# AKASH2907/pi-consistency-activity-detection

Hardware: AMD Instinct MI355X
Metric: train clips/sec (bs=8, 16×224×224, I3D+caps+bv cons) at 1/2/4/8 GPU (higher is better)
Workload: dtype f32 (fp32 operands and fp32 accumulation everywhere; 33 of the 79 conv / input-gradient launches and the 3x3x3 / 1x1x1 weight gradients multiply on the bf16 matrix cores: every fp32 operand as the exact sum of 3 bf16 terms, 6 products on v_mfma_f32_32x32x16_bf16, hi / lo fp32 accumulators -- error v

## Files before the change

pi-consistency-activity-detection_amd/csrc/caps.hip:

```cpp
#include "common.h"
#include <stdlib.h>

namespace {

constexpr int NB = 32;
constexpr int MAXC = 24;
constexpr int CJ = MAXC / 4;
constexpr float EPS = 1e-8f;
constexpr float LAMBDA = 1e-6f;
constexpr float HALF_LN_2PI = 0.91893853320467274178f;

#define WSYNC()                                               \
    do {                                                      \
        __builtin_amdgcn_fence(__ATOMIC_RELEASE, "workgroup"); \
        __builtin_amdgcn_wave_barrier();                      \
        __builtin_amdgcn_fence(__ATOMIC_ACQUIRE, "workgroup"); \
    } while (0)

template <int CTRL> __device__ __forceinline__ float dpp_mov(float v) {
    return __builtin_bit_cast(float, __builtin_amdgcn_update_dpp(0, __builtin_bit_cast(int, v), CTRL, 0xf, 0xf, true));
}
constexpr int DPP_XOR1 = 0xB1, DPP_XOR2 = 0x4E;
constexpr int DPP_HALF_MIRROR = 0x141, DPP_MIRROR = 0x140;
constexpr int DPP_ROR4 = 0x124, DPP_ROR8 = 0x128;
// ... 496 lines not shown
                    if (t < 2) is2[t][j] = 0.f;
                    if (c < C) {
                        dm[t][j] = bs->dmu[t][c][h]; dsv[t][j] = bs->ds2[t][c][h]; muv[t][j] = st->mu[t][c][h];
                        irs[t][j] = 1.0f / (st->rs[t][c] + EPS);
                        if (t < 2) is2[t][j] = 1.0f / st->s2[t][c][h];
                    }
                }
            float* dxp = dx + pos * (NB * 17);
            for (int i = i0; i < i1; ++i) {
                const f32x4 prow = *(const f32x4*)&st->P[i][p * 4];
                const float ai = st->a[i];
                f32x4 dP = {0.f, 0.f, 0.f, 0.f};
#pragma unroll
                for (int j = 0; j < CJ; ++j) {
                    const int c = cg + 4 * j;
                    if (c >= C) continue;
                    const f32x4 w = *(const f32x4*)(WT + ((i * C + c) * 4 + q) * 4);
                    const float v = prow[0] * w[0] + prow[1] * w[1] + prow[2] * w[2] + prow[3] * w[3];
                    float dv = 0.f;
#pragma unroll
                    for (int t = 0; t < 3; ++t) {
                        const float co = Rt(st, t, i, c, C) * ai * st->invS[t][i] * irs[t][j];
                        dv += co * (dm[t][j] + 2.f * dsv[t][j] * (v - muv[t][j]));
                        if (t < 2) dv -= bs->dlnp[t][i][c] * (v - muv[t][j]) * is2[t][j];
                    }
                    dP += dv * w;
                    f32x4 tk = dv * prow;
#pragma unroll
                    for (int k = 0; k < 4; ++k) tk[k] = sum_p(tk[k]);
                    const float mine = p == 0 ? tk[0] : (p == 1 ? tk[1] : (p == 2 ? tk[2] : tk[3]));
                    if (live) atomicAdd(pp + ((i * C + c) * 4 + p) * 4 + q, mine);
                }
#pragma unroll
                for (int k = 0; k < 4; ++k) {
                    dP[k] = sum_cg(add_xor2(add_xor1(dP[k])));
                }
                if (q == 0 && cg == 0 && live) *(f32x4*)(dxp + i * 16 + p * 4) = dP;
            }
            if (tid < NB && live) dxp[NB * 16 + tid] = bs->da_in[tid];
        }
    }
    __syncthreads();
    for (int e = tid; e < EM_SMALL; e += NT) pp[NB * MAXC * 16 + e] = dbu[e];
}

constexpr int RED_E = 32, RED_S = 8;
__global__ __launch_bounds__(256) void em_reduce_kernel(const float* __restrict__ part, int nblk, int C, float* dW, float* dbu, float* dba) {
    __shared__ double sh[RED_S][RED_E];
    const int stride = NB * MAXC * 16 + MAXC * 16 + 32;
    const int nW = NB * C * 16, nU = C * 16;
    const int el = threadIdx.x % RED_E, sl = threadIdx.x / RED_E;
    const int e = blockIdx.x * RED_E + el;
    const bool act = e < nW + nU + C;
    int src = 0; float* dst = nullptr;
    if (act) {
        if (e < nW) { src = e; dst = dW + e; }
        else if (e < nW + nU) { src = NB * MAXC * 16 + (e - nW); dst = dbu + (e - nW); }
        else { src = NB * MAXC * 16 + MAXC * 16 + (e - nW - nU); dst = dba + (e - nW - nU); }
    }
    double s = 0.0;
    if (act) {
        int b = sl;
        for (; b + 7 * RED_S < nblk; b += 8 * RED_S) {
            float v[8];
#pragma unroll
            for (int q = 0; q < 8; ++q) v[q] = part[(size_t)(b + q * RED_S) * stride + src];
#pragma unroll
            for (int q = 0; q < 8; ++q) s += (double)v[q];
        }
        for (; b < nblk; b += RED_S) s += (double)part[(size_t)b * stride + src];
    }
    sh[sl][el] = s;
    __syncthreads();
    if (sl == 0 && act) {
        double t = sh[0][el];
#pragma unroll
        for (int q = 1; q < RED_S; ++q) t += sh[q][el];
        *dst += (float)t;
    }
}

__global__ __launch_bounds__(256) void cmask_pred_kernel(const float* __restrict__ caps, int npos, int C, const float* __restrict__ cls,
                                                         const int* __restrict__ labeled, int mode, float* __restrict__ pred, float* __restrict__ mask) {
    __shared__ float sh[256];
    __shared__ float pr[MAXC];
    const int b = blockIdx.x;
    const float* cb = caps + (size_t)b * npos * C * 17 + C * 16;
    for (int c = 0; c < C; ++c) {
        float s = 0.f;
        for (int i = threadIdx.x; i < npos; i += 256) s += cb[(size_t)i * C * 17 + c];
        sh[threadIdx.x] = s;
        __syncthreads();
        for (int o = 128; o > 0; o >>= 1) { if (threadIdx.x < o) sh[threadIdx.x] += sh[threadIdx.x + o]; __syncthreads(); }
        if (threadIdx.x == 0) { pr[c] = sh[0] / npos; pred[b * C + c] = pr[c]; }
        __syncthreads();
    }
    if (threadIdx.x == 0) {
        int am = 0;
        for (int c = 1; c < C; ++c) if (pr[c] > pr[am]) am = c;
        const bool lab = mode != 2 && labeled[b] != 0;
        const int gt = (int)cls[b];
        for (int c = 0; c < C; ++c) {
            float m;
            if (lab) m = c == gt ? 1.f : 0.f;
            else if (mode == 0) m = 1.f;
            else m = c == am ? 1.f : 0.f;
            mask[b * C + c] = m;
        }
    }
}

__global__ __launch_bounds__(256) void cmask_apply_kernel(const float* __restrict__ caps, const float* __restrict__ mask, int npos, int C,
                                                          int64_t total, float* __restrict__ masked) {
    const int PC = C * 16;
    for (int64_t idx = (int64_t)blockIdx.x * 256 + threadIdx.x; idx < total; idx += (int64_t)gridDim.x * 256) {
        const int64_t row = idx / PC; const int e = (int)(idx - row * PC);
        const int b = (int)(row / npos);
        masked[idx] = caps[row * (C * 17) + e] * mask[b * C + (e >> 4)];
    }
}

__global__ __launch_bounds__(256) void cmask_bwd_kernel(const float* __restrict__ dmasked, const float* __restrict__ dpred, const float* __restrict__ mask,
                                                        int npos, int C, int64_t total, float* __restrict__ dcaps) {
    const int W17 = C * 17, PC = C * 16;
    for (int64_t idx = (int64_t)blockIdx.x * 256 + threadIdx.x; idx < total; idx += (int64_t)gridDim.x * 256) {
        const int64_t row = idx / W17; const int e = (int)(idx - row * W17);
        const int b = (int)(row / npos);
        float v;
        if (e < PC) v = dmasked[row * PC + e] * mask[b * C + (e >> 4)];
        else v = dpred ? dpred[b * C + (e - PC)] / npos : 0.f;
        dcaps[idx] = v;
    }
}

constexpr int TS_H = 8, TS_W = 32, TS_LD = 13;
__global__ __launch_bounds__(256) void tapsum_fwd_kernel(const float* __restrict__ proj, int N, int T, int H, int W, const float* __restrict__ bias,
                                                         float* __restrict__ out) {
    __shared__ float slab[(TS_H + 2) * (TS_W + 2) * TS_LD];
    const int wt = (W + TS_W - 1) / TS_W, ht = (H + TS_H - 1) / TS_H;
    int bid = blockIdx.x;
    const int w0 = (bid % wt) * TS_W; bid /= wt;
    const int h0 = (bid % ht) * TS_H; bid /= ht;
    const int t = bid % T; const int n = bid / T;
    const int hl = threadIdx.x / TS_W, wl = threadIdx.x % TS_W;
    float s = bias ? bias[0] : 0.f;
    for (int a = 0; a < 3; ++a) {
        const int ti = t + 1 - a;
        if ((unsigned)ti >= (unsigned)T) continue;
        const int f0 = (9 * a) / 4;
        __syncthreads();
        for (int e = threadIdx.x; e < (TS_H + 2) * (TS_W + 2) * 3; e += 256) {
            const int pos = e / 3, f = e - pos * 3;
            const int r = pos / (TS_W + 2), c = pos - r * (TS_W + 2);
            const int hi = h0 - 1 + r, wi = w0 - 1 + c;
            f32x4 v = {0.f, 0.f, 0.f, 0.f};
            if ((unsigned)hi < (unsigned)H && (unsigned)wi < (unsigned)W)
                v = *(const f32x4*)(proj + ((size_t)((n * T + ti) * H + hi) * W + wi) * 32 + (f0 + f) * 4);
            float* d = slab + pos * TS_LD + f * 4;
            d[0] = v[0]; d[1] = v[1]; d[2] = v[2]; d[3] = v[3];
        }
        __syncthreads();
        const int k0 = 9 * a - 4 * f0;
#pragma unroll
        for (int b = 0; b < 3; ++b)
#pragma unroll
            for (int c = 0; c < 3; ++c)
                s += slab[((hl + 2 - b) * (TS_W + 2) + (wl + 2 - c)) * TS_LD + k0 + 3 * b + c];
    }
    const int h = h0 + hl, w = w0 + wl;
    if (h < H && w < W) out[(size_t)((n * T + t) * H + h) * W + w] = s;
}

__global__ __launch_bounds__(256) void tapsum_bwd_kernel(const float* __restrict__ dout, int N, int T, int H, int W, float* __restrict__ dproj) {
    const int64_t total = (int64_t)N * T * H * W * 8;
    for (int64_t idx = (int64_t)blockIdx.x * 256 + threadIdx.x; idx < total; idx += (int64_t)gridDim.x * 256) {
        int64_t r = idx >> 3; const int g4 = (int)(idx & 7);
        const int64_t pos = r;
        const int w = (int)(r % W); r /= W;
        const int h = (int)(r % H); r /= H;
// ... 103 lines not shown
```

pi-consistency-activity-detection_amd/csrc/spectral.hip:

```cpp
#include "common.h"

namespace {

struct AxK {
    const float* in; const float* M; const float* bias; float* out;
    int R, I, O, C4;
    int in_split, out_split, act, act_c0, accum;
    int in_sr, in_hi, in_lo, out_sr, out_hi, out_lo;
};

constexpr int AX_OC = 8;

__global__ __launch_bounds__(256) void axis_linear_kernel(const AxK p) {
    extern __shared__ float Ms[];
    for (int k = threadIdx.x; k < p.O * p.I; k += 256) Ms[k] = p.M[k];
    __syncthreads();
    const int64_t idx = (int64_t)blockIdx.x * 256 + threadIdx.x;
    if (idx >= (int64_t)p.R * p.C4) return;
    const int r = (int)(idx / p.C4), c = (int)(idx - (int64_t)r * p.C4) * 4;
    const float* ip = p.in + (int64_t)r * p.in_sr + c;
    float* op = p.out + (int64_t)r * p.out_sr + c;
    float4 b = make_float4(0.f, 0.f, 0.f, 0.f);
    if (p.bias) b = *(const float4*)(p.bias + c);
    {
        const int o0 = blockIdx.y * AX_OC;
        float4 acc[AX_OC];
#pragma unroll
        for (int q = 0; q < AX_OC; ++q) acc[q] = make_float4(0.f, 0.f, 0.f, 0.f);
        for (int i = 0; i < p.I; ++i) {
            const float4 v = *(const float4*)(ip + (int64_t)(i / p.in_split) * p.in_hi + (int64_t)(i % p.in_split) * p.in_lo);
#pragma unroll
            for (int q = 0; q < AX_OC; ++q) {
                const float m = (o0 + q < p.O) ? Ms[(o0 + q) * p.I + i] : 0.f;
                acc[q].x += m * v.x; acc[q].y += m * v.y; acc[q].z += m * v.z; acc[q].w += m * v.w;
            }
        }
#pragma unroll
        for (int q = 0; q < AX_OC; ++q) {
            const int o = o0 + q;
            if (o >= p.O) break;
            float* dst = op + (int64_t)(o / p.out_split) * p.out_hi + (int64_t)(o % p.out_split) * p.out_lo;
            float4 y = acc[q];
            y.x += b.x; y.y += b.y; y.z += b.z; y.w += b.w;
            if (p.accum) {
                const float4 old = *(const float4*)dst;
                y.x += old.x; y.y += old.y; y.z += old.z; y.w += old.w;
            }
            if (p.act == PC_ACT_SIGMOID && c >= p.act_c0) {
                y.x = 1.f / (1.f + expf(-y.x)); y.y = 1.f / (1.f + expf(-y.y));
                y.z = 1.f / (1.f + expf(-y.z)); y.w = 1.f / (1.f + expf(-y.w));
            } else if (p.act == PC_ACT_RELU && c >= p.act_c0) {
                y.x = fmaxf(y.x, 0.f); y.y = fmaxf(y.y, 0.f); y.z = fmaxf(y.z, 0.f); y.w = fmaxf(y.w, 0.f);
            }
            *(float4*)dst = y;
        }
    }
}

constexpr int WS_MAXK = 16;

template <int KX>
__global__ __launch_bounds__(256) void wspec_fwd_kernel(const float* __restrict__ in, const float* __restrict__ tw, int A, int B4, int KY,
                                                         int U, int Ur, float* __restrict__ out) {
    const int64_t idx = (int64_t)blockIdx.x * 256 + threadIdx.x;
    if (idx >= (int64_t)A * KY * B4) return;
    const int b = (int)(idx % B4) * 4;
    const int ky = (int)((idx / B4) % KY);
    const int a = (int)(idx / ((int64_t)B4 * KY));
    const int B = B4 * 4;
    float4 v[KX];
#pragma unroll
    for (int kx = 0; kx < KX; ++kx) v[kx] = *(const float4*)(in + ((int64_t)a * KY * KX + ky * KX + kx) * B + b);
    const int64_t plane = (int64_t)A * KY * B;
    float* o = out + ((int64_t)a * KY + ky) * B + b;
    for (int u = 0; u < U; ++u) {
        float4 wr = make_float4(0.f, 0.f, 0.f, 0.f), wi = wr;
#pragma unroll
        for (int kx = 0; kx < KX; ++kx) {
            const float c = tw[(u * KX + kx) * 2], s = tw[(u * KX + kx) * 2 + 1];
            wr.x += c * v[kx].x; wr.y += c * v[kx].y; wr.z += c * v[kx].z; wr.w += c * v[kx].w;
            wi.x += s * v[kx].x; wi.y += s * v[kx].y; wi.z += s * v[kx].z; wi.w += s * v[kx].w;
        }
        if (u >= U - Ur) { *(float4*)(o + (int64_t)(3 * (U - Ur) + u - (U - Ur)) * plane) = wr; continue; }
        float* ou = o + (int64_t)u * 3 * plane;
        *(float4*)ou = wr;
        *(float4*)(ou + plane) = make_float4(wr.x - wi.x, wr.y - wi.y, wr.z - wi.z, wr.w - wi.w);
        *(float4*)(ou + 2 * plane) = make_float4(wr.x + wi.x, wr.y + wi.y, wr.z + wi.z, wr.w + wi.w);
    }
}

template <int KX>
__global__ __launch_bounds__(256) void wspec_bwd_kernel(const float* __restrict__ dV, const float* __restrict__ tw, int A, int B4, int KY,
                                                         int U, int Ur, float* __restrict__ kg) {
    const int64_t idx = (int64_t)blockIdx.x * 256 + threadIdx.x;
    if (idx >= (int64_t)A * KY * B4) return;
    const int b = (int)(idx % B4) * 4;
    const int ky = (int)((idx / B4) % KY);
    const int a = (int)(idx / ((int64_t)B4 * KY));
    const int B = B4 * 4;
    float4 acc[KX];
#pragma unroll
    for (int kx = 0; kx < KX; ++kx) acc[kx] = make_float4(0.f, 0.f, 0.f, 0.f);
    const int64_t plane = (int64_t)A * KY * B;
    const float* d = dV + ((int64_t)a * KY + ky) * B + b;
    for (int u = U - Ur; u < U; ++u) {
        const float4 d0 = *(const float4*)(d + (int64_t)(3 * (U - Ur) + u - (U - Ur)) * plane);
#pragma unroll
        for (int kx = 0; kx < KX; ++kx) {
            const float c = tw[(u * KX + kx) * 2];
            acc[kx].x += c * d0.x; acc[kx].y += c * d0.y; acc[kx].z += c * d0.z; acc[kx].w += c * d0.w;
        }
    }
#pragma unroll 5
    for (int u = 0; u < U - Ur; ++u) {
        const float* du = d + (int64_t)u * 3 * plane;
        const float4 d0 = *(const float4*)du, d1 = *(const float4*)(du + plane), d2 = *(const float4*)(du + 2 * plane);
        const float4 gr = make_float4(d0.x + d1.x + d2.x, d0.y + d1.y + d2.y, d0.z + d1.z + d2.z, d0.w + d1.w + d2.w);
        const float4 gi = make_float4(d2.x - d1.x, d2.y - d1.y, d2.z - d1.z, d2.w - d1.w);
#pragma unroll
// ... 175 lines not shown
```

pi-consistency-activity-detection_amd/csrc/tail.hip:

```cpp
#include "common.h"

namespace {

constexpr int J32 = 32;

__global__ __launch_bounds__(256) void tail_combine_kernel(const float* __restrict__ W4, const float* __restrict__ b4, const float* __restrict__ cs,
                                                           const float* __restrict__ Wp, int N, int Ci, int Co, int taps, int J,
                                                           float* __restrict__ Wt, float* __restrict__ Wf, float* __restrict__ bc) {
    const int64_t total = (int64_t)N * Ci * taps * J32;
    for (int64_t idx = (int64_t)blockIdx.x * 256 + threadIdx.x; idx < total; idx += (int64_t)gridDim.x * 256) {
        const int j = (int)(idx & 31);
        int64_t r = idx >> 5;
        const int tap = (int)(r % taps); r /= taps;
        const int ci = (int)(r % Ci); const int n = (int)(r / Ci);
        float acc = 0.f;
        if (j < J) {
            const float* w4 = W4 + (size_t)ci * Co * taps + tap;
            for (int co = 0; co < Co; ++co) {
                const float sc = cs ? cs[n * Co + co] : 1.f;
                acc += w4[(size_t)co * taps] * sc * Wp[co * J + j];
            }
        }
        Wt[idx] = acc;
        Wf[(((size_t)n * J32 + j) * taps + tap) * Ci + ci] = acc;
    }
    if (blockIdx.x == 0) {
        for (int e = threadIdx.x; e < N * J32; e += 256) {
            const int n = e >> 5, j = e & 31;
            float acc = 0.f;
            if (j < J)
                for (int co = 0; co < Co; ++co) acc += b4[co] * (cs ? cs[n * Co + co] : 1.f) * Wp[co * J + j];
            bc[e] = acc;
        }
    }
}

__global__ __launch_bounds__(256) void tail_colsum_kernel(const float* __restrict__ dproj, int64_t rows_per_n, int64_t rows_per_block, float* __restrict__ s) {
    __shared__ float sh[8][32];
    const int n = blockIdx.y, j = threadIdx.x & 31, rl = threadIdx.x >> 5;
    const int64_t r0 = (int64_t)blockIdx.x * rows_per_block, r1 = min(rows_per_n, r0 + rows_per_block);
    const float* base = dproj + (size_t)n * rows_per_n * J32;
    float acc = 0.f;
    for (int64_t r = r0 + rl; r < r1; r += 8) acc += base[r * J32 + j];
    sh[rl][j] = acc;
    __syncthreads();
    if (rl == 0) {
        float t = 0.f;
        for (int q = 0; q < 8; ++q) t += sh[q][j];
        atomicAdd(s + n * J32 + j, t);
    }
}

constexpr int DW4_MAXN = 64;
__global__ __launch_bounds__(128) void tail_dw4_kernel(const float* __restrict__ G, const float* __restrict__ cs, const float* __restrict__ Wp,
                                                       int N, int Ci, int Co, int taps, int J, float* __restrict__ dW4, int accum) {
    __shared__ float g[DW4_MAXN][J32];
    const int ci = blockIdx.x / taps, tap = blockIdx.x - ci * taps;
    for (int e = threadIdx.x; e < N * J32; e += 128) g[e >> 5][e & 31] = G[(((size_t)(e >> 5) * Ci + ci) * taps + tap) * J32 + (e & 31)];
    __syncthreads();
    for (int co = threadIdx.x; co < Co; co += 128) {
        float wp[J32];
#pragma unroll
        for (int j = 0; j < J32; ++j) wp[j] = j < J ? Wp[co * J + j] : 0.f;
        float acc = 0.f;
        for (int n = 0; n < N; ++n) {
            float a = 0.f;
#pragma unroll
            for (int j = 0; j < J32; ++j) a += g[n][j] * wp[j];
            acc += (cs ? cs[n * Co + co] : 1.f) * a;
        }
        const size_t idx = ((size_t)ci * Co + co) * taps + tap;
        dW4[idx] = (accum ? dW4[idx] : 0.f) + acc;
    }
}

constexpr int DWP_CI = 8;
__global__ __launch_bounds__(256) void tail_dwp_kernel(const float* __restrict__ G, const float* __restrict__ W4, const float* __restrict__ cs,
                                                       int Ci, int Co, int taps, int J, float* __restrict__ dWp, float* __restrict__ part) {
    extern __shared__ float gs[];
    const int n = blockIdx.y, ci0 = blockIdx.x * DWP_CI;
    const int rows = DWP_CI * taps;
    const float* gsrc = G + ((size_t)n * Ci + ci0) * taps * J32;
    for (int e = threadIdx.x; e < rows * J32; e += 256) gs[e] = gsrc[e];
    __syncthreads();
    const int half = threadIdx.x & 1;
    float* pb = part ? part + ((size_t)n * gridDim.x + blockIdx.x) * Co * J32 : nullptr;
    for (int co = threadIdx.x >> 1; co < Co; co += 128) {
        float acc[16];
#pragma unroll
        for (int q = 0; q < 16; ++q) acc[q] = 0.f;
        for (int r = 0; r < rows; ++r) {
            const int ci = ci0 + r / taps, tap = r - (r / taps) * taps;
            const float w = W4[((size_t)ci * Co + co) * taps + tap];
            const float* gr = gs + r * J32 + half * 16;
#pragma unroll
            for (int q = 0; q < 16; ++q) acc[q] += w * gr[q];
        }
        const float sc = cs ? cs[n * Co + co] : 1.f;
        if (pb) {
#pragma unroll
            for (int q = 0; q < 16; q += 4) *(float4*)(pb + co * J32 + half * 16 + q) = make_float4(sc * acc[q], sc * acc[q + 1], sc * acc[q + 2], sc * acc[q + 3]);
            continue;
        }
#pragma unroll
        for (int q = 0; q < 16; ++q) {
            const int j = half * 16 + q;
            if (j < J) atomicAdd(dWp + co * J + j, sc * acc[q]);
        }
    }
}

__global__ __launch_bounds__(256) void tail_dwp_sum_kernel(const float* __restrict__ part, int np, int Co, int J, float* __restrict__ dWp, int accum) {
    const int e = blockIdx.x * 256 + threadIdx.x;
    if (e >= Co * J32) return;
    const int co = e / J32, j = e - co * J32;
    const size_t st = (size_t)Co * J32;
    float v = 0.f;
    int q = 0;
    for (; q + 16 <= np; q += 16) {
        float t[16];
#pragma unroll
        for (int u = 0; u < 16; ++u) t[u] = part[(size_t)(q + u) * st + e];
#pragma unroll
        for (int u = 0; u < 16; ++u) v += t[u];
    }
    for (; q < np; ++q) v += part[(size_t)q * st + e];
    if (j < J) dWp[co * J + j] = (accum ? dWp[co * J + j] : 0.f) + v;
}

__global__ __launch_bounds__(64) void tail_dbias_kernel(const float* __restrict__ s, const float* __restrict__ b4, const float* __restrict__ cs,
                                                        const float* __restrict__ Wp, int N, int Co, int J, int center, float* __restrict__ dWp,
                                                        float* __restrict__ db4, float* __restrict__ dbp, int accum) {
    const int co = blockIdx.x, j = threadIdx.x & 31;
    if (threadIdx.x >= 32) return;
    float sb = 0.f;
    for (int n = 0; n < N; ++n) sb += (cs ? cs[n * Co + co] : 1.f) * s[n * J32 + j];
    if (j < J) dWp[co * J + j] += b4[co] * sb;
    float v = j < J ? Wp[co * J + j] * sb : 0.f;
#pragma unroll
    for (int o = 16; o > 0; o >>= 1) v += __shfl_xor(v, o, 64);
    if (j == 0) db4[co] = (accum ? db4[co] : 0.f) + v;
    if (co == 0 && j == 0) {
        float t2 = 0.f;
        for (int n = 0; n < N; ++n) t2 += s[n * J32 + center];
        dbp[0] = (accum ? dbp[0] : 0.f) + t2;
    }
}

}

extern "C" int pc_tail_combine(const float* W4, const float* b4, const float* cs, const float* Wp, int N, int Ci, int Co, int taps, int J,
                               float* Wt, float* Wf, float* bc, pc_stream s) {
    PC_CHECK_ARG(W4 && b4 && Wp && Wt && Wf && bc && J <= J32 && N >= 1, "pc_tail_combine: bad args");
    const int64_t total = (int64_t)N * Ci * taps * J32;
    int grid = (int)((total + 255) / 256); if (grid > 8192) grid = 8192;
    hipLaunchKernelGGL(tail_combine_kernel, dim3(grid), dim3(256), 0, (hipStream_t)s, W4, b4, cs, Wp, N, Ci, Co, taps, J, Wt, Wf, bc);
    PC_CHECK_LAUNCH("tail_combine");
    return PC_OK;
}

extern "C" int pc_tail_colsum(const float* dproj, int N, int64_t rows_per_n, float* sums, pc_stream s_) {
    hipStream_t s = (hipStream_t)s_;
    PC_CHECK_ARG(dproj && sums && N >= 1 && N <= 65535, "pc_tail_colsum: bad args");
    (void)hipMemsetAsync(sums, 0, sizeof(float) * N * J32, s);
    int64_t rpb = (rows_per_n + 255) / 256; if (rpb < 64) rpb = 64;
    const int nb = (int)((rows_per_n + rpb - 1) / rpb);
    hipLaunchKernelGGL(tail_colsum_kernel, dim3(nb, N), dim3(256), 0, s, dproj, rows_per_n, rpb, sums);
    PC_CHECK_LAUNCH("tail_colsum");
    return PC_OK;
}

extern "C" int64_t pc_tail_grads_ws_floats(int N, int Ci, int Co) {
    if (N < 1 || Ci < DWP_CI || Ci % DWP_CI || Co < 1) return -1;
    return (int64_t)N * (Ci / DWP_CI) * Co * J32;
}

extern "C" int pc_tail_grads_ws(const float* G, const float* sums, const float* W4, const float* b4, const float* cs, const float* Wp, int N,
                                int Ci, int Co, int taps, int J, int center, float* dW4, float* db4, float* dWp, float* dbp, int accum, float* ws,
                                pc_stream s_) {
    hipStream_t s = (hipStream_t)s_;
    PC_CHECK_ARG(G && sums && W4 && b4 && Wp && dW4 && db4 && dWp && dbp && J <= J32, "pc_tail_grads: bad args");
    PC_CHECK_ARG(N <= DW4_MAXN && Ci % DWP_CI == 0, "pc_tail_grads: N <= %d and Ci %% %d == 0 expected (N=%d Ci=%d)", DW4_MAXN, DWP_CI, N, Ci);
    hipLaunchKernelGGL(tail_dw4_kernel, dim3(Ci * taps), dim3(128), 0, s, G, cs, Wp, N, Ci, Co, taps, J, dW4, accum);
    if (!ws && !accum) (void)hipMemsetAsync(dWp, 0, sizeof(float) * Co * J, s);
    hipLaunchKernelGGL(tail_dwp_kernel, dim3(Ci / DWP_CI, N), dim3(256), (size_t)DWP_CI * taps * J32 * 4, s, G, W4, cs, Ci, Co, taps, J, dWp, ws);
    if (ws) hipLaunchKernelGGL(tail_dwp_sum_kernel, dim3((Co * J32 + 255) / 256), dim3(256), 0, s, ws, N * (Ci / DWP_CI), Co, J, dWp, accum);
    hipLaunchKernelGGL(tail_dbias_kernel, dim3(Co), dim3(64), 0, s, sums, b4, cs, Wp, N, Co, J, center, dWp, db4, dbp, accum);
    PC_CHECK_LAUNCH("tail_grads");
    return PC_OK;
}

extern "C" int pc_tail_grads(const float* G, const float* sums, const float* W4, const float* b4, const float* cs, const float* Wp, int N,
                             int Ci, int Co, int taps, int J, int center, float* dW4, float* db4, float* dWp, float* dbp, int accum, pc_stream s) {
    return pc_tail_grads_ws(G, sums, W4, b4, cs, Wp, N, Ci, Co, taps, J, center, dW4, db4, dWp, dbp, accum, nullptr, s);
}
```

pi-consistency-activity-detection_amd/csrc/tail6.hip:

```cpp
#include "common.h"
#include <stdlib.h>

namespace {

constexpr int NSLOT = 125, SP = 128, J32 = 32;

__device__ __forceinline__ int npairs(int k5, bool first) { return k5 == 0 || k5 == 4 ? 1 : (k5 == 2 ? (first ? 2 : 3) : 2); }
__device__ __forceinline__ int pair_k4(int k5, bool first, int q) {
    switch (k5) {
        case 0: return 0;
        case 1: return q;
        case 2: return first ? 1 + q : q;
        case 3: return 1 + q;
        default: return 2;
    }
}

__global__ __launch_bounds__(256) void tail6_weights_kernel(const float* __restrict__ wf, int N, int Ci, float* __restrict__ W5f,
                                                            float* __restrict__ W5t) {
    const int64_t total = (int64_t)N * 8 * SP * Ci;
    for (int64_t idx = (int64_t)blockIdx.x * 256 + threadIdx.x; idx < total; idx += (int64_t)gridDim.x * 256) {
        const int ci = (int)(idx % Ci);
        const int slot = (int)((idx / Ci) % SP);
        const int z = (int)((idx / ((int64_t)Ci * SP)) % 8);
        const int n = (int)(idx / ((int64_t)Ci * SP * 8));
        float acc = 0.f;
        if (slot < NSLOT) {
            const int st = slot / 25, sh = (slot / 5) % 5, sw = slot % 5;
            const bool ft = z & 4, fh = z & 2, fw = z & 1;
            const float* base = wf + (size_t)n * J32 * 27 * Ci + ci;
            for (int a = 0; a < npairs(st, ft); ++a)
                for (int b = 0; b < npairs(sh, fh); ++b)
                    for (int c = 0; c < npairs(sw, fw); ++c) {
                        const int ka = pair_k4(st, ft, a), kb = pair_k4(sh, fh, b), kc = pair_k4(sw, fw, c);
                        const int tap = (ka * 3 + kb) * 3 + kc;
                        const int j = ((st - ka) * 3 + (sh - kb)) * 3 + (sw - kc);
                        acc += base[((size_t)j * 27 + tap) * Ci];
                    }
        }
        W5f[idx] = acc;
        W5t[(((size_t)n * 8 + z) * Ci + ci) * SP + slot] = acc;
    }
}

__device__ __forceinline__ int dim_terms(int o, int I, int (&ii)[3], int (&kk)[3]) {
    int n = 0;
#pragma unroll
    for (int k5 = 0; k5 < 5; ++k5) {
        const int t = o + 2 - k5;
        if (t >= 0 && !(t & 1) && (t >> 1) < I) { ii[n] = t >> 1; kk[n] = k5; ++n; }
    }
    return n;
}

__global__ __launch_bounds__(256) void tail6_gather_kernel(const float* __restrict__ cols, const float* __restrict__ bc, const float* __restrict__ bsm,
                                                           int N, int It, int Ih, int Iw, float* __restrict__ out) {
    const int Ot = 2 * It, Oh = 2 * Ih, Ow = 2 * Iw;
    const int64_t total = (int64_t)N * Ot * Oh * Ow;
    const int64_t idx = (int64_t)blockIdx.x * 256 + threadIdx.x;
    if (idx >= total) return;
    const int ow = (int)(idx % Ow), oh = (int)((idx / Ow) % Oh), ot = (int)((idx / ((int64_t)Ow * Oh)) % Ot), n = (int)(idx / ((int64_t)Ow * Oh * Ot));
    int it[3], kt[3], ih[3], kh[3], iw[3], kw[3];
    const int nt = dim_terms(ot, It, it, kt), nh = dim_terms(oh, Ih, ih, kh), nw = dim_terms(ow, Iw, iw, kw);
    float acc = bsm[0];
    for (int a = 0; a < 3; ++a) {
        const int mt = ot + 1 - a;
        if (mt < 0 || mt >= Ot) continue;
        for (int b = 0; b < 3; ++b) {
            const int mh = oh + 1 - b;
            if (mh < 0 || mh >= Oh) continue;
            for (int c = 0; c < 3; ++c) {
                const int mw = ow + 1 - c;
                if (mw < 0 || mw >= Ow) continue;
                acc += bc[n * J32 + (a * 3 + b) * 3 + c];
            }
        }
    }
    const size_t P3 = (size_t)It * Ih * Iw;
    const float* base = cols + (size_t)n * SP * P3;
    for (int a = 0; a < nt; ++a)
        for (int b = 0; b < nh; ++b) {
            const size_t pos = ((size_t)it[a] * Ih + ih[b]) * Iw;
            const int slot0 = (kt[a] * 5 + kh[b]) * 5;
            for (int c = 0; c < nw; ++c) acc += base[(size_t)(slot0 + kw[c]) * P3 + pos + iw[c]];
        }
    out[idx] = acc;
}

template <int PT, int PH>
__global__ __launch_bounds__(128) void tail6_gather_rows_kernel(const float* __restrict__ cols, const float* __restrict__ bc, const float* __restrict__ bsm,
                                                                int N, int It, int Ih, int Iw, float* __restrict__ out) {
    __shared__ float sbc[28];
    const int Ot = 2 * It, Oh = 2 * Ih, Ow = 2 * Iw;
    int row = blockIdx.x;
    const int qh = row % Ih; row /= Ih;
    const int qt = row % It; const int n = row / It;
    const int ot = 2 * qt + PT, oh = 2 * qh + PH;
    if (threadIdx.x < 27) sbc[threadIdx.x] = bc[n * J32 + threadIdx.x];
    __syncthreads();
    if (threadIdx.x == 0) { float t = 0.f; for (int e = 0; e < 27; ++e) t += sbc[e]; sbc[27] = t; }
    __syncthreads();
    constexpr int NT = PT ? 2 : 3, NH = PH ? 2 : 3;
    const size_t P3 = (size_t)It * Ih * Iw;
    const float* base = cols + (size_t)n * SP * P3;
    const bool tb = ot == 0 || ot == Ot - 1, hb = oh == 0 || oh == Oh - 1;
    for (int qw = threadIdx.x; qw < Iw; qw += 128) {
        float acc0 = 0.f, acc1 = 0.f;
        const int iwp = qw + 1 < Iw ? qw + 1 : qw, iwm = qw >= 1 ? qw - 1 : 0;
        const float fwp = qw + 1 < Iw ? 1.f : 0.f, fwm = qw >= 1 ? 1.f : 0.f;
#pragma unroll
        for (int a = 0; a < NT; ++a) {
            const int it_ = PT ? qt + 1 - a : qt + 1 - a, kt = PT ? 1 + 2 * a : 2 * a;
            const bool vt = it_ >= 0 && it_ < It;
            const int itc = vt ? it_ : 0;
#pragma unroll
            for (int b = 0; b < NH; ++b) {
                const int ih_ = qh + 1 - b, kh = PH ? 1 + 2 * b : 2 * b;
                const bool vh = ih_ >= 0 && ih_ < Ih;
                const int ihc = vh ? ih_ : 0;
                const float f = (vt && vh) ? 1.f : 0.f;
                const float* pl = base + (size_t)((kt * 5 + kh) * 5) * P3 + ((size_t)itc * Ih + ihc) * Iw;
                const float e0 = pl[iwp], e2 = pl[2 * P3 + qw], e4 = pl[4 * P3 + iwm];
                const float o1 = pl[P3 + iwp], o3 = pl[3 * P3 + qw];
                acc0 += f * ((fwp * e0 + e2) + fwm * e4);
// ... 84 lines not shown
    }
}
__global__ __launch_bounds__(256) void tail6_wgrad_map_kernel(const float* __restrict__ dW5, int N, int Ci, float* __restrict__ Gc, const T6Slices sl) {
    const int64_t total = (int64_t)N * Ci * 27 * J32;
    for (int64_t idx = (int64_t)blockIdx.x * 256 + threadIdx.x; idx < total; idx += (int64_t)gridDim.x * 256) {
        const int j = (int)(idx & 31);
        const int tap = (int)((idx >> 5) % 27);
        const int ci = (int)((idx / (27 * J32)) % Ci);
        const int n = (int)(idx / ((int64_t)27 * J32 * Ci));
        float acc = 0.f;
        if (j < 27) {
            const int k4[3] = {tap / 9, (tap / 3) % 3, tap % 3}, ks[3] = {j / 9, (j / 3) % 3, j % 3};
            const int slot = ((k4[0] + ks[0]) * 5 + k4[1] + ks[1]) * 5 + k4[2] + ks[2];
            const bool bad[3] = {k4[0] == 0 && ks[0] == 2, k4[1] == 0 && ks[1] == 2, k4[2] == 0 && ks[2] == 2};
            for (int z = 0; z < 8; ++z) {
                if (((z & 4) && bad[0]) || ((z & 2) && bad[1]) || ((z & 1) && bad[2])) continue;
                if (!sl.image) { acc += dW5[(((size_t)n * 8 + z) * Ci + ci) * SP + slot]; continue; }
                if (sl.n[z]) acc += dW5[sl.zoff[z] + ((size_t)n * Ci + ci) * SP + slot];
            }
        }
        Gc[idx] = acc;
    }
}

__global__ __launch_bounds__(256) void tail6_bias_sums_kernel(const float* __restrict__ dout, int Ot, int Oh, int Ow, int64_t per_block, float* __restrict__ sums,
                                                              float* __restrict__ part) {
    __shared__ float sh[27][8];
    const int n = blockIdx.y;
    const int64_t per_n = (int64_t)Ot * Oh * Ow;
    const int64_t r0 = (int64_t)blockIdx.x * per_block, r1 = min(per_n, r0 + per_block);
    float acc[27];
#pragma unroll
    for (int q = 0; q < 27; ++q) acc[q] = 0.f;
    for (int64_t r = r0 + threadIdx.x; r < r1; r += 256) {
        const int ow = (int)(r % Ow), oh = (int)((r / Ow) % Oh), ot = (int)(r / ((int64_t)Ow * Oh));
        const float v = dout[(size_t)n * per_n + r];
        const float vt[3] = {ot + 1 < Ot ? 1.f : 0.f, 1.f, ot >= 1 ? 1.f : 0.f};
        const float vh[3] = {oh + 1 < Oh ? 1.f : 0.f, 1.f, oh >= 1 ? 1.f : 0.f};
        const float vw[3] = {ow + 1 < Ow ? 1.f : 0.f, 1.f, ow >= 1 ? 1.f : 0.f};
#pragma unroll
        for (int a = 0; a < 3; ++a)
#pragma unroll
            for (int b = 0; b < 3; ++b)
#pragma unroll
                for (int c = 0; c < 3; ++c) acc[(a * 3 + b) * 3 + c] += v * vt[a] * vh[b] * vw[c];
    }
    const int lane = threadIdx.x & 63, wave = threadIdx.x >> 6;
#pragma unroll
    for (int q = 0; q < 27; ++q) {
        float s = acc[q];
        for (int o = 32; o > 0; o >>= 1) s += __shfl_xor(s, o, 64);
        if (lane == 0) sh[q][wave] = s;
    }
    __syncthreads();
    if (threadIdx.x < 27) {
        const float v = sh[threadIdx.x][0] + sh[threadIdx.x][1] + sh[threadIdx.x][2] + sh[threadIdx.x][3];
        if (part) part[((size_t)n * gridDim.x + blockIdx.x) * J32 + threadIdx.x] = v;
        else atomicAdd(sums + n * J32 + threadIdx.x, v);
    }
}

__global__ __launch_bounds__(32) void tail6_bias_sums_final_kernel(const float* __restrict__ part, int nb, float* __restrict__ sums) {
    const int n = blockIdx.x, j = threadIdx.x;
    float v = 0.f;
    if (j < 27) {
        const float* q = part + (size_t)n * nb * J32 + j;
        int b = 0;
        for (; b + 14 <= nb; b += 14) {
            float t[14];
#pragma unroll
            for (int u = 0; u < 14; ++u) t[u] = q[(size_t)(b + u) * J32];
#pragma unroll
            for (int u = 0; u < 14; ++u) v += t[u];
        }
        for (; b < nb; ++b) v += q[(size_t)b * J32];
    }
    sums[n * J32 + j] = v;
}

}

extern "C" int pc_tail6_weights(const float* wf, int N, int Ci, float* W5f, float* W5t, pc_stream s) {
    PC_CHECK_ARG(wf && W5f && W5t && N >= 1 && Ci >= 1, "pc_tail6_weights: bad args");
    const int64_t total = (int64_t)N * 8 * SP * Ci;
    int grid = (int)((total + 255) / 256); if (grid > 8192) grid = 8192;
    hipLaunchKernelGGL(tail6_weights_kernel, dim3(grid), dim3(256), 0, (hipStream_t)s, wf, N, Ci, W5f, W5t);
    PC_CHECK_LAUNCH("tail6_weights");
    return PC_OK;
}

extern "C" int pc_tail6_gather(const float* cols, const float* bc, const float* bsm, int N, int It, int Ih, int Iw, float* out, pc_stream s) {
    PC_CHECK_ARG(cols && bc && bsm && out && N >= 1 && It >= 1 && Ih >= 1 && Iw >= 1, "pc_tail6_gather: bad args");
    const int64_t total = (int64_t)N * 8 * It * Ih * Iw;
    PC_CHECK_ARG((total + 255) / 256 < (1ll << 31), "pc_tail6_gather: too large");
    if (((uintptr_t)out & 7) == 0) {
        const dim3 grid((unsigned)((int64_t)N * It * Ih));
        hipLaunchKernelGGL((tail6_gather_rows_kernel<0, 0>), grid, dim3(128), 0, (hipStream_t)s, cols, bc, bsm, N, It, Ih, Iw, out);
        hipLaunchKernelGGL((tail6_gather_rows_kernel<0, 1>), grid, dim3(128), 0, (hipStream_t)s, cols, bc, bsm, N, It, Ih, Iw, out);
        hipLaunchKernelGGL((tail6_gather_rows_kernel<1, 0>), grid, dim3(128), 0, (hipStream_t)s, cols, bc, bsm, N, It, Ih, Iw, out);
        hipLaunchKernelGGL((tail6_gather_rows_kernel<1, 1>), grid, dim3(128), 0, (hipStream_t)s, cols, bc, bsm, N, It, Ih, Iw, out);
    } else {
        hipLaunchKernelGGL(tail6_gather_kernel, dim3((unsigned)cdiv(total, 256)), dim3(256), 0, (hipStream_t)s, cols, bc, bsm, N, It, Ih, Iw, out);
    }
    PC_CHECK_LAUNCH("tail6_gather");
    return PC_OK;
}

extern "C" int pc_tail6_scatter(const float* dout, int N, int It, int Ih, int Iw, float* dcols, pc_stream s) {
    PC_CHECK_ARG(dout && dcols && N >= 1 && It >= 1 && Ih >= 1 && Iw >= 1, "pc_tail6_scatter: bad args");
    const int64_t total = (int64_t)N * It * Ih * Iw * (SP / 4);
    PC_CHECK_ARG((total + 255) / 256 < (1ll << 31), "pc_tail6_scatter: too large");
    const int64_t nblk = (int64_t)N * It * Ih * cdiv(Iw, SC_RUN);
    PC_CHECK_ARG(nblk < (1ll << 31), "pc_tail6_scatter: too large");
    hipLaunchKernelGGL(tail6_scatter_kernel, dim3((unsigned)nblk), dim3(256), 0, (hipStream_t)s, dout, N, It, Ih, Iw, dcols);
    PC_CHECK_LAUNCH("tail6_scatter");
    return PC_OK;
}

static int t6_wgrad_map(float* dW5, const int32_t* nslices8, int N, int Ci, float* Gc, pc_stream s) {
    PC_CHECK_ARG(dW5 && Gc && N >= 1 && Ci >= 1, "pc_tail6_wgrad_map: bad args");
    T6Slices sl;
    sl.image = nslices8 ? (long long)N * Ci * SP : 0;
    long long at = 0;
    for (int z = 0; z < 8; ++z) {
        sl.n[z] = nslices8 ? nslices8[z] : 1;
        PC_CHECK_ARG(sl.n[z] >= 0 && sl.n[z] <= 65536, "pc_tail6_wgrad_map_slices: class %d has %d slice images", z, sl.n[z]);
        sl.zoff[z] = at;
        at += sl.n[z] * sl.image;
    }
    const int64_t total = (int64_t)N * Ci * 27 * J32;
    int grid = (int)((total + 255) / 256); if (grid > 8192) grid = 8192;
    if (sl.image) {
        int g4 = (int)((sl.image / 4 + 255) / 256); if (g4 > 512) g4 = 512;
        hipLaunchKernelGGL(tail6_slices_sum_kernel, dim3(g4, 8), dim3(256), 0, (hipStream_t)s, dW5, sl);
    }
    hipLaunchKernelGGL(tail6_wgrad_map_kernel, dim3(grid), dim3(256), 0, (hipStream_t)s, dW5, N, Ci, Gc, sl);
    PC_CHECK_LAUNCH("tail6_wgrad_map");
    return PC_OK;
}

extern "C" int pc_tail6_wgrad_map_slices(float* ws, const int32_t* nslices8, int N, int Ci, float* Gc, pc_stream s) {
    PC_CHECK_ARG(nslices8, "pc_tail6_wgrad_map_slices: no slice counts");
    return t6_wgrad_map(ws, nslices8, N, Ci, Gc, s);
}

extern "C" int pc_tail6_wgrad_map(const float* dW5, int N, int Ci, float* Gc, pc_stream s) {
    return t6_wgrad_map(const_cast<float*>(dW5), nullptr, N, Ci, Gc, s);
}

namespace {
inline void t6_bias_blocks(int It, int Ih, int Iw, int64_t& pb, int& nb) {
    const int64_t per_n = (int64_t)8 * It * Ih * Iw;
    pb = (per_n + 255) / 256; if (pb < 4096) pb = 4096;
    nb = (int)((per_n + pb - 1) / pb);
}
}

extern "C" int64_t pc_tail6_bias_sums_ws_floats(int N, int It, int Ih, int Iw) {
    if (N < 1 || It < 1 || Ih < 1 || Iw < 1) return -1;
    int64_t pb; int nb;
    t6_bias_blocks(It, Ih, Iw, pb, nb);
    return (int64_t)N * nb * J32;
}

extern "C" int pc_tail6_bias_sums_ws(const float* dout, int N, int It, int Ih, int Iw, float* sums, float* ws, pc_stream s_) {
    hipStream_t s = (hipStream_t)s_;
    PC_CHECK_ARG(dout && sums && N >= 1 && N <= 65535, "pc_tail6_bias_sums: bad args");
    int64_t pb; int nb;
    t6_bias_blocks(It, Ih, Iw, pb, nb);
// ... 11 lines not shown
```

Baseline: 449.9.

## Tile tail weight-combine kernels, batch axis-linear loads, single-pass class mask reduction

Four separate kernel rewrites. tail_combine now stages W4 and Wp chunks in shared memory per block of input channels, keeps register prefetching and per-tap accumulators, and adds a dedicated block for the bias. tail6_weights precomputes per-slot term lists in shared memory and transposes through an LDS tile so both outputs are written coalesced. axis_linear unrolls the input loop by 4 with incremental index math, and cmask_pred reduces all classes in one pass instead of one tree reduction per class. These are all small kernels in a conv-dominated training step, so the overall effect is likely limited, at the cost of more shared memory and register pressure.

```diff
diff --git a/pi-consistency-activity-detection_amd/csrc/caps.hip b/pi-consistency-activity-detection_amd/csrc/caps.hip
--- a/pi-consistency-activity-detection_amd/csrc/caps.hip
+++ b/pi-consistency-activity-detection_amd/csrc/caps.hip
@@ -602,19 +602,32 @@
 
 __global__ __launch_bounds__(256) void cmask_pred_kernel(const float* __restrict__ caps, int npos, int C, const float* __restrict__ cls,
                                                          const int* __restrict__ labeled, int mode, float* __restrict__ pred, float* __restrict__ mask) {
-    __shared__ float sh[256];
+    __shared__ float sh[MAXC][256];
     __shared__ float pr[MAXC];
     const int b = blockIdx.x;
     const float* cb = caps + (size_t)b * npos * C * 17 + C * 16;
-    for (int c = 0; c < C; ++c) {
-        float s = 0.f;
-        for (int i = threadIdx.x; i < npos; i += 256) s += cb[(size_t)i * C * 17 + c];
-        sh[threadIdx.x] = s;
+    float s[MAXC];
+#pragma unroll
+    for (int c = 0; c < MAXC; ++c) s[c] = 0.f;
+    for (int i = threadIdx.x; i < npos; i += 256) {
+        const float* row = cb + (size_t)i * C * 17;
+#pragma unroll
+        for (int c = 0; c < MAXC; ++c) if (c < C) s[c] += row[c];
+    }
+#pragma unroll
+    for (int c = 0; c < MAXC; ++c) if (c < C) sh[c][threadIdx.x] = s[c];
+    __syncthreads();
+    for (int o = 128; o > 0; o >>= 1) {
+        if (threadIdx.x < o) {
+#pragma unroll
+            for (int c = 0; c < MAXC; ++c) if (c < C) s[c] += sh[c][threadIdx.x + o];
+#pragma unroll
+            for (int c = 0; c < MAXC; ++c) if (c < C) sh[c][threadIdx.x] = s[c];
+        }
         __syncthreads();
-        for (int o = 128; o > 0; o >>= 1) { if (threadIdx.x < o) sh[threadIdx.x] += sh[threadIdx.x + o]; __syncthreads(); }
-        if (threadIdx.x == 0) { pr[c] = sh[0] / npos; pred[b * C + c] = pr[c]; }
-        __syncthreads();
-    }
+    }
+    if (threadIdx.x < C) { pr[threadIdx.x] = sh[threadIdx.x][0] / npos; pred[b * C + threadIdx.x] = pr[threadIdx.x]; }
+    __syncthreads();
     if (threadIdx.x == 0) {
         int am = 0;
         for (int c = 1; c < C; ++c) if (pr[c] > pr[am]) am = c;
diff --git a/pi-consistency-activity-detection_amd/csrc/spectral.hip b/pi-consistency-activity-detection_amd/csrc/spectral.hip
--- a/pi-consistency-activity-detection_amd/csrc/spectral.hip
+++ b/pi-consistency-activity-detection_amd/csrc/spectral.hip
@@ -10,6 +10,24 @@
 };
 
 constexpr int AX_OC = 8;
+
+template <int U>
+__device__ __forceinline__ void ax_batch(const AxK& p, const float* Ms, const float* ip, int i0, int o0, int& hi, int& lo, float4 (&acc)[AX_OC]) {
+    float4 v[U];
+#pragma unroll
+    for (int u = 0; u < U; ++u) {
+        v[u] = *(const float4*)(ip + (int64_t)hi * p.in_hi + (int64_t)lo * p.in_lo);
+        if (++lo == p.in_split) { lo = 0; ++hi; }
+    }
+#pragma unroll
+    for (int u = 0; u < U; ++u) {
+#pragma unroll
+        for (int q = 0; q < AX_OC; ++q) {
+            const float m = (o0 + q < p.O) ? Ms[(o0 + q) * p.I + i0 + u] : 0.f;
+            acc[q].x += m * v[u].x; acc[q].y += m * v[u].y; acc[q].z += m * v[u].z; acc[q].w += m * v[u].w;
+        }
+    }
+}
 
 __global__ __launch_bounds__(256) void axis_linear_kernel(const AxK p) {
     extern __shared__ float Ms[];
@@ -27,14 +45,10 @@
         float4 acc[AX_OC];
 #pragma unroll
         for (int q = 0; q < AX_OC; ++q) acc[q] = make_float4(0.f, 0.f, 0.f, 0.f);
-        for (int i = 0; i < p.I; ++i) {
-            const float4 v = *(const float4*)(ip + (int64_t)(i / p.in_split) * p.in_hi + (int64_t)(i % p.in_split) * p.in_lo);
-#pragma unroll
-            for (int q = 0; q < AX_OC; ++q) {
-                const float m = (o0 + q < p.O) ? Ms[(o0 + q) * p.I + i] : 0.f;
-                acc[q].x += m * v.x; acc[q].y += m * v.y; acc[q].z += m * v.z; acc[q].w += m * v.w;
-            }
-        }
+        int i = 0, hi = 0, lo = 0;
+        for (; i + 4 <= p.I; i += 4) ax_batch<4>(p, Ms, ip, i, o0, hi, lo, acc);
+        if (i + 2 <= p.I) { ax_batch<2>(p, Ms, ip, i, o0, hi, lo, acc); i += 2; }
+        if (i < p.I) ax_batch<1>(p, Ms, ip, i, o0, hi, lo, acc);
 #pragma unroll
         for (int q = 0; q < AX_OC; ++q) {
             const int o = o0 + q;
diff --git a/pi-consistency-activity-detection_amd/csrc/tail.hip b/pi-consistency-activity-detection_amd/csrc/tail.hip
--- a/pi-consistency-activity-detection_amd/csrc/tail.hip
+++ b/pi-consistency-activity-detection_amd/csrc/tail.hip
@@ -4,7 +4,110 @@
 
 constexpr int J32 = 32;
 
+constexpr int TC_CI = 8, TC_CK = 32, TC_CKP = TC_CK + 4, TC_TAPS = 27, TC_SM = (TC_CK * TC_TAPS + 255) / 256;
+
+constexpr int TCB_CO = 128;
+__device__ __forceinline__ void tail_combine_bias(const float* __restrict__ b4, const float* __restrict__ cs, const float* __restrict__ Wp, int n, int Co, int J,
+                                                  float* __restrict__ bc, float* wpl, float* bsc) {
+    float a = 0.f;
+    for (int cb = 0; cb < Co; cb += TCB_CO) {
+        const int m = min(TCB_CO, Co - cb);
+        __syncthreads();
+        for (int e = threadIdx.x; e < m; e += 256) bsc[e] = b4[cb + e] * (cs ? cs[n * Co + cb + e] : 1.f);
+        for (int e = threadIdx.x; e < m * J; e += 256) wpl[e] = Wp[cb * J + e];
+        __syncthreads();
+        if (threadIdx.x < J) {
+#pragma unroll 8
+            for (int q = 0; q < m; ++q) a += bsc[q] * wpl[q * J + threadIdx.x];
+        }
+    }
+    if (threadIdx.x < J32) bc[n * J32 + threadIdx.x] = a;
+}
+
 __global__ __launch_bounds__(256) void tail_combine_kernel(const float* __restrict__ W4, const float* __restrict__ b4, const float* __restrict__ cs,
+                                                           const float* __restrict__ Wp, int N, int Ci, int Co, int taps, int J,
+                                                           float* __restrict__ Wt, float* __restrict__ Wf, float* __restrict__ bc) {
+    __shared__ __attribute__((aligned(16))) float w4s[TC_CI * TC_TAPS * TC_CKP];
+    __shared__ float wps[TC_CK * J32];
+    const int n = blockIdx.y, ci0 = blockIdx.x * TC_CI;
+    if (ci0 >= Ci) { tail_combine_bias(b4, cs, Wp, n, Co, J, bc, w4s, wps); return; }
+    const int cil = threadIdx.x >> 5, j = threadIdx.x & 31;
+    float acc[TC_TAPS];
+#pragma unroll
+    for (int k = 0; k < TC_TAPS; ++k) acc[k] = 0.f;
+    int soff[TC_SM], scc[TC_SM];
+#pragma unroll
+    for (int m = 0; m < TC_SM; ++m) {
+        const int e = threadIdx.x + 256 * m, cc = e / taps;
+        scc[m] = cc; soff[m] = (e - cc * taps) * TC_CKP + cc;
+    }
+    float wr[TC_CI][TC_SM], scr[TC_SM], pr[TC_CK * J32 / 256];
+    auto fetch = [&](int co0) {
+        const int cn = min(TC_CK, Co - co0), slab = cn * taps;
+#pragma unroll
+        for (int m = 0; m < TC_SM; ++m) {
+            const int e = threadIdx.x + 256 * m;
+            const bool ok = e < slab;
+            scr[m] = (ok && cs) ? cs[n * Co + co0 + scc[m]] : 1.f;
+#pragma unroll
+            for (int l = 0; l < TC_CI; ++l) wr[l][m] = (ok && ci0 + l < Ci) ? W4[((size_t)(ci0 + l) * Co + co0) * taps + e] : 0.f;
+        }
+#pragma unroll
+        for (int u = 0; u < TC_CK * J32 / 256; ++u) {
+            const int e = threadIdx.x + 256 * u, cc = e >> 5, jj = e & 31;
+            pr[u] = (cc < cn && jj < J) ? Wp[(co0 + cc) * J + jj] : 0.f;
+        }
+    };
+    fetch(0);
+    for (int co0 = 0; co0 < Co; co0 += TC_CK) {
+        const int cn = min(TC_CK, Co - co0), slab = cn * taps;
+        __syncthreads();
+        if (cn < TC_CK) {
+            for (int e = threadIdx.x; e < TC_CI * TC_TAPS * TC_CKP; e += 256) w4s[e] = 0.f;
+            __syncthreads();
+        }
+#pragma unroll
+        for (int m = 0; m < TC_SM; ++m) {
+            if (threadIdx.x + 256 * m < slab) {
+#pragma unroll
+                for (int l = 0; l < TC_CI; ++l) w4s[l * TC_TAPS * TC_CKP + soff[m]] = wr[l][m] * scr[m];
+            }
+        }
+#pragma unroll
+        for (int u = 0; u < TC_CK * J32 / 256; ++u) wps[threadIdx.x + 256 * u] = pr[u];
+        __syncthreads();
+        if (co0 + TC_CK < Co) fetch(co0 + TC_CK);
+        const float* wrow = w4s + cil * TC_TAPS * TC_CKP;
+        for (int cc = 0; cc < TC_CK; cc += 4) {
+            const float p0 = wps[cc * J32 + j], p1 = wps[(cc + 1) * J32 + j], p2 = wps[(cc + 2) * J32 + j], p3 = wps[(cc + 3) * J32 + j];
+#pragma unroll
+            for (int k = 0; k < TC_TAPS; ++k) {
+                if (k < taps) {
+                    const f32x4 w = *(const f32x4*)(wrow + k * TC_CKP + cc);
+                    acc[k] += w[0] * p0; acc[k] += w[1] * p1; acc[k] += w[2] * p2; acc[k] += w[3] * p3;
+                }
+            }
+        }
+    }
+    const bool live = ci0 + cil < Ci;
+    if (live) {
+        float* wt = Wt + (((size_t)n * Ci + ci0 + cil) * taps) * J32 + j;
+#pragma unroll
+        for (int k = 0; k < TC_TAPS; ++k) if (k < taps) wt[(size_t)k * J32] = j < J ? acc[k] : 0.f;
+    }
+    __syncthreads();
+#pragma unroll
+    for (int k = 0; k < TC_TAPS; ++k) if (k < taps) w4s[(j * TC_TAPS + k) * TC_CI + cil] = j < J ? acc[k] : 0.f;
+    __syncthreads();
+    const int cw = min(TC_CI, Ci - ci0);
+    for (int e = threadIdx.x; e < J32 * taps * TC_CI; e += 256) {
+        const int l = e % TC_CI, jt = e / TC_CI;
+        const int jj = jt / taps, tap = jt - jj * taps;
+        if (l < cw) Wf[(((size_t)n * J32 + jj) * taps + tap) * Ci + ci0 + l] = w4s[(jj * TC_TAPS + tap) * TC_CI + l];
+    }
+}
+
+__global__ __launch_bounds__(256) void tail_combine_generic_kernel(const float* __restrict__ W4, const float* __restrict__ b4, const float* __restrict__ cs,
                                                            const float* __restrict__ Wp, int N, int Ci, int Co, int taps, int J,
                                                            float* __restrict__ Wt, float* __restrict__ Wf, float* __restrict__ bc) {
     const int64_t total = (int64_t)N * Ci * taps * J32;
@@ -154,7 +257,10 @@
     PC_CHECK_ARG(W4 && b4 && Wp && Wt && Wf && bc && J <= J32 && N >= 1, "pc_tail_combine: bad args");
     const int64_t total = (int64_t)N * Ci * taps * J32;
     int grid = (int)((total + 255) / 256); if (grid > 8192) grid = 8192;
-    hipLaunchKernelGGL(tail_combine_kernel, dim3(grid), dim3(256), 0, (hipStream_t)s, W4, b4, cs, Wp, N, Ci, Co, taps, J, Wt, Wf, bc);
+    if (taps >= 1 && taps <= TC_TAPS && Ci >= 1 && Co >= 1 && N <= 65535)
+        hipLaunchKernelGGL(tail_combine_kernel, dim3((unsigned)cdiv(Ci, TC_CI) + 1, (unsigned)N), dim3(256), 0, (hipStream_t)s, W4, b4, cs, Wp, N, Ci, Co, taps, J, Wt, Wf, bc);
+    else
+        hipLaunchKernelGGL(tail_combine_generic_kernel, dim3(grid), dim3(256), 0, (hipStream_t)s, W4, b4, cs, Wp, N, Ci, Co, taps, J, Wt, Wf, bc);
     PC_CHECK_LAUNCH("tail_combine");
     return PC_OK;
 }
diff --git a/pi-consistency-activity-detection_amd/csrc/tail6.hip b/pi-consistency-activity-detection_amd/csrc/tail6.hip
--- a/pi-consistency-activity-detection_amd/csrc/tail6.hip
+++ b/pi-consistency-activity-detection_amd/csrc/tail6.hip
@@ -16,30 +16,52 @@
     }
 }
 
+constexpr int T6_SL = 32, T6_CI = 32, T6_NT = 27;
 __global__ __launch_bounds__(256) void tail6_weights_kernel(const float* __restrict__ wf, int N, int Ci, float* __restrict__ W5f,
                                                             float* __restrict__ W5t) {
-    const int64_t total = (int64_t)N * 8 * SP * Ci;
-    for (int64_t idx = (int64_t)blockIdx.x * 256 + threadIdx.x; idx < total; idx += (int64_t)gridDim.x * 256) {
-        const int ci = (int)(idx % Ci);
-        const int slot = (int)((idx / Ci) % SP);
-        const int z = (int)((idx / ((int64_t)Ci * SP)) % 8);
-        const int n = (int)(idx / ((int64_t)Ci * SP * 8));
-        float acc = 0.f;
+    __shared__ int nterm[T6_SL];
+    __shared__ int term[T6_SL][T6_NT];
+    __shared__ float tile[T6_SL][T6_CI + 1];
+    const int slot0 = (blockIdx.x % (SP / T6_SL)) * T6_SL, c0 = (blockIdx.x / (SP / T6_SL)) * T6_CI, z = blockIdx.y, n = blockIdx.z;
+    if (threadIdx.x < T6_SL) {
+        const int slot = slot0 + threadIdx.x;
+        int nt = 0;
         if (slot < NSLOT) {
             const int st = slot / 25, sh = (slot / 5) % 5, sw = slot % 5;
             const bool ft = z & 4, fh = z & 2, fw = z & 1;
-            const float* base = wf + (size_t)n * J32 * 27 * Ci + ci;
             for (int a = 0; a < npairs(st, ft); ++a)
                 for (int b = 0; b < npairs(sh, fh); ++b)
                     for (int c = 0; c < npairs(sw, fw); ++c) {
                         const int ka = pair_k4(st, ft, a), kb = pair_k4(sh, fh, b), kc = pair_k4(sw, fw, c);
                         const int tap = (ka * 3 + kb) * 3 + kc;
                         const int j = ((st - ka) * 3 + (sh - kb)) * 3 + (sw - kc);
-                        acc += base[((size_t)j * 27 + tap) * Ci];
+                        term[threadIdx.x][nt++] = j * 27 + tap;
                     }
         }
-        W5f[idx] = acc;
-        W5t[(((size_t)n * 8 + z) * Ci + ci) * SP + slot] = acc;
+        nterm[threadIdx.x] = nt;
+    }
+    const float* base = wf + (size_t)n * J32 * 27 * Ci;
+    float* of = W5f + (((size_t)n * 8 + z) * SP + slot0) * Ci;
+    float* ot = W5t + ((size_t)n * 8 + z) * Ci * SP + slot0;
+    {
+        const int cw = min(T6_CI, Ci - c0);
+        __syncthreads();
+        for (int e = threadIdx.x; e < T6_SL * cw; e += 256) {
+            const int sl = e / cw, ci = c0 + e - sl * cw;
+            const int nt = nterm[sl];
+            float v[T6_NT], acc = 0.f;
+#pragma unroll
+            for (int q = 0; q < T6_NT; ++q) v[q] = q < nt ? base[(size_t)term[sl][q] * Ci + ci] : 0.f;
+#pragma unroll
+            for (int q = 0; q < T6_NT; ++q) if (q < nt) acc += v[q];
+            of[(size_t)sl * Ci + ci] = acc;
+            tile[sl][ci - c0] = acc;
+        }
+        __syncthreads();
+        for (int e = threadIdx.x; e < T6_SL * cw; e += 256) {
+            const int cl = e / T6_SL, sl = e % T6_SL;
+            ot[(size_t)(c0 + cl) * SP + sl] = tile[sl][cl];
+        }
     }
 }
 
@@ -290,9 +312,7 @@
 
 extern "C" int pc_tail6_weights(const float* wf, int N, int Ci, float* W5f, float* W5t, pc_stream s) {
     PC_CHECK_ARG(wf && W5f && W5t && N >= 1 && Ci >= 1, "pc_tail6_weights: bad args");
-    const int64_t total = (int64_t)N * 8 * SP * Ci;
-    int grid = (int)((total + 255) / 256); if (grid > 8192) grid = 8192;
-    hipLaunchKernelGGL(tail6_weights_kernel, dim3(grid), dim3(256), 0, (hipStream_t)s, wf, N, Ci, W5f, W5t);
+    hipLaunchKernelGGL(tail6_weights_kernel, dim3((SP / T6_SL) * (unsigned)cdiv(Ci, T6_CI), 8, (unsigned)N), dim3(256), 0, (hipStream_t)s, wf, N, Ci, W5f, W5t);
     PC_CHECK_LAUNCH("tail6_weights");
     return PC_OK;
 }
```

New measurement: 451.9 (median of 6 runs). About the same (+0.4%).
